# sehyun03/MulActSeg

Hardware: AMD Instinct MI355X
Metric: superpixels scored/sec (higher is better)
Workload: dtype f32; 1 GPU; acquisition-round: PixBal+ban-ignore scorer on resident logits, Cityscapes pool shape [4,20,1024,2048] per step; per rank K single-pass scans (class prior + region sums + histograms) of its shard, then exchange 1 (all-gather class sums) + device class weights (k_class_weight) + weighted finalize + ban + exchange 2 (all-gather scores) + replicated K4 (keys, radix sort, fair-counting budget walk) ov; nseg=2048, id_dtype=int64, regions_scored=679936, budget_clicks=11159, regions_selected=6688

## Files before the change

mulactseg_amd/csrc/single_pass.hip:

```cpp
#include <cstdlib>
#include "common.h"

namespace {

constexpr int kThreads = 256;
constexpr int kTileW = 256;
constexpr int kTileH = 16;
constexpr int kLogSlots = 7;
constexpr int kSlots = 1 << kLogSlots;

__device__ __forceinline__ int table_slot(int* keys, int id) {
    unsigned h = ((unsigned)id * 2654435769u) >> (32 - kLogSlots);
    for (int probe = 0; probe < kSlots; ++probe) {
        int k = __hip_atomic_load(&keys[h], __ATOMIC_RELAXED, __HIP_MEMORY_SCOPE_WORKGROUP);
        if (k == id) return (int)h;
        if (k == -1) {
            int old = atomicCAS(&keys[h], -1, id);
            if (old == -1 || old == id) return (int)h;
        }
        h = (h + 1) & (kSlots - 1);
    }
    return -1;
}

struct LowSrc { int h, w; float sh, sw; };
constexpr int kLowRows = 7, kLowCols = 68;

__device__ __forceinline__ void low_tap(float scale, int o, int& i0, float& l0, float& l1) {
    float s = scale * ((float)o + 0.5f) - 0.5f;
    s = s < 0.0f ? 0.0f : s;
    i0 = (int)s;
    l1 = s - (float)i0;
    l0 = 1.0f - l1;
}

template <int CT, bool EXACT, typename IdT, bool VEC, bool LOWRES = false, bool X4 = false>
__global__ __launch_bounds__(kThreads) void k_single_pass(const float* __restrict__ z, const IdT* __restrict__ spx, int C, int H,
                                                           int W, int S, float invT, int tiles_x, int tiles_y,
                                                           mas_u64* __restrict__ prob_sum, mas_u64* __restrict__ class_sum,
                                                           unsigned* __restrict__ hist, const LowSrc lr = LowSrc{0, 0, 0.f, 0.f}) {
    extern __shared__ __attribute__((aligned(16))) unsigned char smem[];
    mas_u64* t_sum = reinterpret_cast<mas_u64*>(smem);
    mas_u64* s_part = reinterpret_cast<mas_u64*>(smem + sizeof(mas_u64) * kSlots * C);
    unsigned* t_hist = reinterpret_cast<unsigned*>(smem + sizeof(mas_u64) * (kSlots * C + 4 * CT));
    int* t_keys = reinterpret_cast<int*>(smem + sizeof(mas_u64) * (kSlots * C + 4 * CT) + sizeof(unsigned) * kSlots * C);
    float* s_low = reinterpret_cast<float*>(t_keys + kSlots);

    for (int i = threadIdx.x; i < kSlots; i += kThreads) t_keys[i] = -1;
    for (int i = threadIdx.x; i < kSlots * C; i += kThreads) { t_sum[i] = 0; t_hist[i] = 0; }

    int bid = blockIdx.x;
    const int tx = bid % tiles_x; bid /= tiles_x;
    const int ty = bid % tiles_y;
    const int b = bid / tiles_y;
    const int HW = H * W;
    const float* zb = z + (size_t)b * C * (LOWRES ? lr.h * lr.w : HW);
    int low_r0 = 0, low_c0 = 0;
    if (LOWRES) {
        float u0, u1;
        low_tap(lr.sh, ty * kTileH, low_r0, u0, u1);
        low_tap(lr.sw, tx * kTileW, low_c0, u0, u1);
        const int lane_ = threadIdx.x & (MAS_WAVE - 1), wave_ = threadIdx.x / MAS_WAVE;
        for (int cr = wave_; cr < C * kLowRows; cr += kThreads / MAS_WAVE) {
            const int c = cr / kLowRows, r = cr - c * kLowRows;
            const int gy = min(low_r0 + r, lr.h - 1);
            const float* src = zb + ((size_t)c * lr.h + gy) * lr.w;
            for (int x = lane_; x < kLowCols; x += MAS_WAVE) s_low[cr * kLowCols + x] = src[min(low_c0 + x, lr.w - 1)];
        }
    }
    __syncthreads();
    const IdT* sb = spx + (size_t)b * HW;
    mas_u64* gsum = class_sum + (size_t)b * S * C;
    unsigned* ghist = hist + (size_t)b * S * C;
    const int lane = threadIdx.x & (MAS_WAVE - 1);
    const int wave = threadIdx.x / MAS_WAVE;

    unsigned acc[CT];
#pragma unroll
    for (int c = 0; c < CT; ++c) acc[c] = 0;
    unsigned n_quanta = 0;
    int lx[4];
    mas_v2f l0xa = mas_splat(0.f), l1xa = mas_splat(0.f), l0xb = mas_splat(0.f), l1xb = mas_splat(0.f);
    if (LOWRES) {
        float a0[4], a1[4];
#pragma unroll
        for (int k = 0; k < 4; ++k) {
            const int xk = tx * kTileW + (VEC ? (lane * 4 + k) : (k * MAS_WAVE + lane));
            int i0;
            low_tap(lr.sw, xk < W ? xk : W - 1, i0, a0[k], a1[k]);
            lx[k] = i0 - low_c0;
        }
        l0xa = (mas_v2f){a0[0], a0[1]}; l1xa = (mas_v2f){a1[0], a1[1]};
        l0xb = (mas_v2f){a0[2], a0[3]}; l1xb = (mas_v2f){a1[2], a1[3]};
    }

    for (int it = 0; it < kTileH / 4; ++it) {
        const int y = ty * kTileH + it * 4 + wave;
        if (y >= H) break;
        const size_t row = (size_t)y * W;
        int xs[4];
        bool ok[4];
#pragma unroll
        for (int k = 0; k < 4; ++k) {
            xs[k] = tx * kTileW + (VEC ? (lane * 4 + k) : (k * MAS_WAVE + lane));
            ok[k] = xs[k] < W;
        }
        int id[4];
#pragma unroll
        for (int k = 0; k < 4; ++k) {
            id[k] = ok[k] ? mas_load_id(sb, row + xs[k]) : -1;
            if (id[k] >= S) id[k] = -1;
        }
        mas_v2f v[2][CT];
        float b1[4], b2[4];
        int a1[4];
#pragma unroll
        for (int k = 0; k < 4; ++k) { b1[k] = -__builtin_inff(); b2[k] = -__builtin_inff(); a1[k] = 0; }
        int ly = 0;
        mas_v2f l0y = mas_splat(0.f), l1y = mas_splat(0.f);
        if (LOWRES) {
            float u0, u1;
            low_tap(lr.sh, y, ly, u0, u1);
            ly -= low_r0;
            l0y = mas_splat(u0);
            l1y = mas_splat(u1);
        }
        if (LOWRES) {
            if constexpr (X4) {
                mas_v2f raw[2][4];
                auto fetch4 = [&](int c, mas_v2f (&d)[4]) {
                    const float* r0 = s_low + (c * kLowRows + ly) * kLowCols;
                    const float* r1 = r0 + kLowCols;
                    d[0] = (mas_v2f){r0[lx[0]], r0[lx[0] + 1]}; d[1] = (mas_v2f){r1[lx[0]], r1[lx[0] + 1]};
                    d[2] = (mas_v2f){r0[lx[2]], r0[lx[2] + 1]}; d[3] = (mas_v2f){r1[lx[2]], r1[lx[2] + 1]};
                };
                const mas_v2f ly01 = {l0y.x, l1y.x};
                fetch4(0, raw[0]);
#pragma unroll
                for (int c = 0; c < CT; ++c) {
                    if (EXACT || c < C) {
                        if (c + 1 < CT && (EXACT || c + 1 < C)) fetch4(c + 1, raw[(c + 1) & 1]);
                        const mas_v2f (&d)[4] = raw[c & 1];
                        v[0][c] = mas_pk_mul_lo(ly01, mas_pk_mul_lo(d[0], l0xa) + mas_pk_mul_hi(d[0], l1xa))
                                + mas_pk_mul_hi(ly01, mas_pk_mul_lo(d[1], l0xa) + mas_pk_mul_hi(d[1], l1xa));
                        v[1][c] = mas_pk_mul_lo(ly01, mas_pk_mul_lo(d[2], l0xb) + mas_pk_mul_hi(d[2], l1xb))
                                + mas_pk_mul_hi(ly01, mas_pk_mul_lo(d[3], l0xb) + mas_pk_mul_hi(d[3], l1xb));
                    }
                }
            } else {
                float raw[2][16];
                auto fetch16 = [&](int c, float (&d)[16]) {
                    const float* r0 = s_low + (c * kLowRows + ly) * kLowCols;
                    const float* r1 = r0 + kLowCols;
#pragma unroll
                    for (int k = 0; k < 4; ++k) {
                        d[4 * k] = r0[lx[k]]; d[4 * k + 1] = r0[lx[k] + 1]; d[4 * k + 2] = r1[lx[k]]; d[4 * k + 3] = r1[lx[k] + 1];
                    }
                };
                fetch16(0, raw[0]);
#pragma unroll
                for (int c = 0; c < CT; ++c) {
                    if (EXACT || c < C) {
                        if (c + 1 < CT && (EXACT || c + 1 < C)) fetch16(c + 1, raw[(c + 1) & 1]);
                        const float (&d)[16] = raw[c & 1];
                        const mas_v2f v00a = {d[0], d[4]}, v01a = {d[1], d[5]}, v10a = {d[2], d[6]}, v11a = {d[3], d[7]};
                        const mas_v2f v00b = {d[8], d[12]}, v01b = {d[9], d[13]}, v10b = {d[10], d[14]}, v11b = {d[11], d[15]};
                        v[0][c] = l0y * (l0xa * v00a + l1xa * v01a) + l1y * (l0xa * v10a + l1xa * v11a);
                        v[1][c] = l0y * (l0xb * v00b + l1xb * v01b) + l1y * (l0xb * v10b + l1xb * v11b);
                    }
                }
            }
        }
#pragma unroll
        for (int c = 0; c < CT; ++c) {
            if (EXACT || c < C) {
                float4 t = make_float4(0.f, 0.f, 0.f, 0.f);
                const float* zc = zb + (size_t)c * HW;
                if (LOWRES) {
                    t = make_float4(v[0][c].x, v[0][c].y, v[1][c].x, v[1][c].y);
                } else if (VEC) {
                    if (ok[0]) t = mas_load_stream4(zc + (unsigned)(row + xs[0]));
                } else {
                    if (ok[0]) t.x = zc[row + xs[0]];
                    if (ok[1]) t.y = zc[row + xs[1]];
                    if (ok[2]) t.z = zc[row + xs[2]];
                    if (ok[3]) t.w = zc[row + xs[3]];
                }
                v[0][c] = (mas_v2f){t.x, t.y};
                v[1][c] = (mas_v2f){t.z, t.w};
                const float q[4] = {t.x, t.y, t.z, t.w};
#pragma unroll
                for (int k = 0; k < 4; ++k) {
                    const bool g1 = q[k] > b1[k];
                    b2[k] = __builtin_amdgcn_fmed3f(b1[k], b2[k], q[k]);
                    a1[k] = g1 ? c : a1[k];
                    b1[k] = __builtin_amdgcn_fmed3f(b1[k], q[k], 3.402823466e+38f);
                }
            } else {
                v[0][c] = mas_splat(0.f);
                v[1][c] = mas_splat(0.f);
            }
        }
        __builtin_amdgcn_sched_barrier(0);
        {
            mas_v2f Ra, Rb;
            mas_softmax_quad<CT, EXACT, true>(v[0], v[1], C, invT, Ra, Rb, (mas_v2f){b1[0], b1[1]}, (mas_v2f){b1[2], b1[3]});
            Ra = Ra * mas_splat(8388608.0f);
            Rb = Rb * mas_splat(8388608.0f);
            Ra = (mas_v2f){ok[0] ? Ra.x : 0.0f, ok[1] ? Ra.y : 0.0f};
            Rb = (mas_v2f){ok[2] ? Rb.x : 0.0f, ok[3] ? Rb.y : 0.0f};
#pragma unroll
            for (int c = 0; c < CT; ++c) {
                if (EXACT || c < C) {
                    const mas_v2f ta = mas_pk_fma(v[0][c], Ra, mas_splat(8388608.0f));
                    const mas_v2f tb = mas_pk_fma(v[1][c], Rb, mas_splat(8388608.0f));
                    acc[c] += (mas_f2u(ta.x) + mas_f2u(ta.y)) + (mas_f2u(tb.x) + mas_f2u(tb.y));
                }
            }
        }
        __builtin_amdgcn_sched_barrier(0);
        n_quanta += 4;
        mas_u64 q[4];
        int key[4];
        float margin[4];
        mas_bvsb_quad(b1, b2, invT, margin);
#pragma unroll
        for (int k = 0; k < 4; ++k) {
            q[k] = mas_fix_unit(margin[k]);
            key[k] = id[k] < 0 ? -1 : id[k] * MAS_MAX_CLASSES + a1[k];
        }
        const bool same = (key[0] == key[1]) && (key[1] == key[2]) && (key[2] == key[3]);
        if (same) {
            if (key[0] >= 0) {
                const int s = table_slot(t_keys, id[0]);
                const mas_u64 qs = (q[0] + q[1]) + (q[2] + q[3]);
                if (s >= 0) {
                    lds_add(&t_sum[s * C + a1[0]], qs);
                    lds_add(&t_hist[s * C + a1[0]], 4u);
                } else {
                    atomicAdd(&gsum[(size_t)id[0] * C + a1[0]], qs);
                    atomicAdd(&ghist[(size_t)id[0] * C + a1[0]], 4u);
                }
            }
        } else {
#pragma unroll
            for (int k = 0; k < 4; ++k) {
                if (key[k] < 0) continue;
                const int s = table_slot(t_keys, id[k]);
                if (s >= 0) {
                    lds_add(&t_sum[s * C + a1[k]], q[k]);
                    lds_add(&t_hist[s * C + a1[k]], 1u);
                } else {
                    atomicAdd(&gsum[(size_t)id[k] * C + a1[k]], q[k]);
                    atomicAdd(&ghist[(size_t)id[k] * C + a1[k]], 1u);
                }
            }
        }
    }

#pragma unroll
    for (int c = 0; c < CT; ++c) {
        mas_u64 a = acc[c] - n_quanta * MAS_PROBQ_BIAS;
#pragma unroll
        for (int off = MAS_WAVE / 2; off > 0; off >>= 1) a += __shfl_down(a, off, MAS_WAVE);
        if (lane == 0) s_part[wave * CT + c] = a;
    }
    __syncthreads();
    if (threadIdx.x < CT && (EXACT || (int)threadIdx.x < C)) {
        mas_u64 a = 0;
#pragma unroll
        for (int w = 0; w < kThreads / MAS_WAVE; ++w) a += s_part[w * CT + threadIdx.x];
        if (a) atomicAdd(&prob_sum[(size_t)b * C + threadIdx.x], a);
    }
    for (int i = threadIdx.x; i < kSlots * C; i += kThreads) {
        const unsigned n = t_hist[i];
        if (n) {
            const int s = i / C;
            const size_t g = (size_t)t_keys[s] * C + (i - s * C);
            atomicAdd(&ghist[g], n);
            atomicAdd(&gsum[g], t_sum[i]);
        }
    }
}

constexpr int kRingTileH = 64;
constexpr int kRingRows = kRingTileH / 4;

template <typename IdT> struct IdQuad;
template <> struct IdQuad<long long> {
    int4 a, b;
    __device__ __forceinline__ void load(const long long* p) {
        a = *reinterpret_cast<const int4*>(p);
        b = *reinterpret_cast<const int4*>(p + 2);
    }
    __device__ __forceinline__ void get(int (&id)[4]) const {
        id[0] = a.y == 0 ? a.x : -1;
        id[1] = a.w == 0 ? a.z : -1;
        id[2] = b.y == 0 ? b.x : -1;
        id[3] = b.w == 0 ? b.z : -1;
    }
};
template <> struct IdQuad<int> {
    int4 a;
    __device__ __forceinline__ void load(const int* p) { a = *reinterpret_cast<const int4*>(p); }
    __device__ __forceinline__ void get(int (&id)[4]) const { id[0] = a.x; id[1] = a.y; id[2] = a.z; id[3] = a.w; }
};
template <> struct IdQuad<unsigned short> {
    uint2 a;
    __device__ __forceinline__ void load(const unsigned short* p) { a = *reinterpret_cast<const uint2*>(p); }
    __device__ __forceinline__ void get(int (&id)[4]) const {
        id[0] = (int)(a.x & 0xffffu); id[1] = (int)(a.x >> 16); id[2] = (int)(a.y & 0xffffu); id[3] = (int)(a.y >> 16);
    }
};

template <int CT, typename IdT>
struct RowRegs {
    float4 t[CT];
    IdQuad<IdT> ids;
};

template <int CT, bool EXACT, typename IdT>
__device__ __forceinline__ void ring_issue(RowRegs<CT, IdT>& r, const float* __restrict__ zb, const IdT* __restrict__ sb, int C,
                                           int HW, unsigned off) {
    r.ids.load(sb + off);
#pragma unroll
    for (int c = 0; c < CT; ++c) {
        if (EXACT || c < C) r.t[c] = mas_load_stream4(zb + (size_t)c * HW + off);
        else r.t[c] = make_float4(0.f, 0.f, 0.f, 0.f);
    }
}

template <int CT, bool EXACT, typename IdT>
__device__ __forceinline__ void ring_consume(RowRegs<CT, IdT>& r, bool ok, int C, int S, float invT, unsigned* s_acc, int* t_keys,
                                             mas_u64* t_sum, unsigned* t_hist, mas_u64* __restrict__ gsum,
                                             unsigned* __restrict__ ghist, int& last_id, int& last_slot) {
    mas_v2f v[2][CT];
    float b1[4], b2[4];
    int a1[4];
#pragma unroll
    for (int k = 0; k < 4; ++k) { b1[k] = -__builtin_inff(); b2[k] = -__builtin_inff(); a1[k] = 0; }
#pragma unroll
    for (int c = 0; c < CT; ++c) {
        if (EXACT || c < C) {
            const float4 t = r.t[c];
            v[0][c] = (mas_v2f){t.x, t.y};
            v[1][c] = (mas_v2f){t.z, t.w};
            const float q[4] = {t.x, t.y, t.z, t.w};
#pragma unroll
            for (int k = 0; k < 4; ++k) {
                const bool g1 = q[k] > b1[k];
                b2[k] = __builtin_amdgcn_fmed3f(b1[k], b2[k], q[k]);
                a1[k] = g1 ? c : a1[k];
                b1[k] = __builtin_amdgcn_fmed3f(b1[k], q[k], 3.402823466e+38f);
            }
        } else {
            v[0][c] = mas_splat(0.f);
            v[1][c] = mas_splat(0.f);
        }
    }
    __builtin_amdgcn_sched_barrier(0);
    {
        mas_v2f Ra, Rb;
        mas_softmax_quad<CT, EXACT, true>(v[0], v[1], C, invT, Ra, Rb, (mas_v2f){b1[0], b1[1]}, (mas_v2f){b1[2], b1[3]});
        Ra = Ra * mas_splat(8388608.0f);
        Rb = Rb * mas_splat(8388608.0f);
        Ra = ok ? Ra : mas_splat(0.0f);
        Rb = ok ? Rb : mas_splat(0.0f);
#pragma unroll
        for (int c = 0; c < CT; ++c) {
            if (EXACT || c < C) {
                const mas_v2f ta = mas_pk_fma(v[0][c], Ra, mas_splat(8388608.0f));
                const mas_v2f tb = mas_pk_fma(v[1][c], Rb, mas_splat(8388608.0f));
                lds_add(&s_acc[c * kThreads + threadIdx.x], (mas_f2u(ta.x) + mas_f2u(ta.y)) + (mas_f2u(tb.x) + mas_f2u(tb.y)));
            }
        }
    }
    __builtin_amdgcn_sched_barrier(0);
    mas_u64 q[4];
    int key[4], id[4];
    float margin[4];
    r.ids.get(id);
    mas_bvsb_quad(b1, b2, invT, margin);
#pragma unroll
    for (int k = 0; k < 4; ++k) {
        id[k] = (ok && id[k] >= 0 && id[k] < S) ? id[k] : -1;
        q[k] = mas_fix_unit(margin[k]);
        key[k] = id[k] < 0 ? -1 : id[k] * MAS_MAX_CLASSES + a1[k];
    }
    const bool same = (key[0] == key[1]) && (key[1] == key[2]) && (key[2] == key[3]);
    if (same) {
        if (key[0] >= 0) {
            if (id[0] != last_id) {
                last_slot = table_slot(t_keys, id[0]);
                last_id = id[0];
            }
            const int s = last_slot;
            const mas_u64 qs = (q[0] + q[1]) + (q[2] + q[3]);
            if (s >= 0) {
                lds_add(&t_sum[s * C + a1[0]], qs);
                lds_add(&t_hist[s * C + a1[0]], 4u);
            } else {
                atomicAdd(&gsum[(size_t)id[0] * C + a1[0]], qs);
                atomicAdd(&ghist[(size_t)id[0] * C + a1[0]], 4u);
            }
        }
    } else {
#pragma unroll
        for (int k = 0; k < 4; ++k) {
            if (key[k] < 0) continue;
            const int s = table_slot(t_keys, id[k]);
            if (s >= 0) {
                lds_add(&t_sum[s * C + a1[k]], q[k]);
                lds_add(&t_hist[s * C + a1[k]], 1u);
            } else {
                atomicAdd(&gsum[(size_t)id[k] * C + a1[k]], q[k]);
                atomicAdd(&ghist[(size_t)id[k] * C + a1[k]], 1u);
            }
        }
    }
}

template <int CT, bool EXACT, typename IdT>
__global__ __launch_bounds__(kThreads, 2) void k_single_pass_ring(const float* __restrict__ z, const IdT* __restrict__ spx, int C,
                                                                   int H, int W, int S, float invT, int tiles_x, int tiles_y,
                                                                   mas_u64* __restrict__ prob_sum,
                                                                   mas_u64* __restrict__ class_sum, unsigned* __restrict__ hist) {
    extern __shared__ __attribute__((aligned(16))) unsigned char smem[];
    mas_u64* t_sum = reinterpret_cast<mas_u64*>(smem);
    mas_u64* s_part = reinterpret_cast<mas_u64*>(smem + sizeof(mas_u64) * kSlots * C);
    unsigned* t_hist = reinterpret_cast<unsigned*>(smem + sizeof(mas_u64) * (kSlots * C + 4 * CT));
    int* t_keys = reinterpret_cast<int*>(smem + sizeof(mas_u64) * (kSlots * C + 4 * CT) + sizeof(unsigned) * kSlots * C);
    unsigned* s_acc = reinterpret_cast<unsigned*>(t_keys + kSlots);

    for (int i = threadIdx.x; i < kSlots; i += kThreads) t_keys[i] = -1;
    for (int i = threadIdx.x; i < kSlots * C; i += kThreads) { t_sum[i] = 0; t_hist[i] = 0; }
#pragma unroll
    for (int c = 0; c < CT; ++c) s_acc[c * kThreads + threadIdx.x] = 0;
    __syncthreads();

    int bid = blockIdx.x;
    const int tx = bid % tiles_x; bid /= tiles_x;
    const int ty = bid % tiles_y;
    const int b = bid / tiles_y;
    const int HW = H * W;
    const float* zb = z + (size_t)b * C * HW;
    const IdT* sb = spx + (size_t)b * HW;
    mas_u64* gsum = class_sum + (size_t)b * S * C;
    unsigned* ghist = hist + (size_t)b * S * C;
    const int lane = threadIdx.x & (MAS_WAVE - 1);
    const int wave = threadIdx.x / MAS_WAVE;

    const int x0 = tx * kTileW + lane * 4;
    const bool okx = x0 < W;
    const unsigned xc = okx ? (unsigned)x0 : 0u;
    const int ybase = ty * kRingTileH + wave;
    auto off_of = [&](int it) -> unsigned {
        int y = ybase + it * 4;
        y = y < H ? y : H - 1;
        return (unsigned)y * (unsigned)W + xc;
    };
    auto ok_of = [&](int it) -> bool { return okx && (ybase + it * 4 < H); };

    RowRegs<CT, IdT> A, B;
    int last_id = -2, last_slot = -1;
    ring_issue<CT, EXACT, IdT>(A, zb, sb, C, HW, off_of(0));
#pragma unroll 1
    for (int it = 0; it < kRingRows; it += 2) {
        ring_issue<CT, EXACT, IdT>(B, zb, sb, C, HW, off_of(it + 1));
        __builtin_amdgcn_sched_barrier(0);
        ring_consume<CT, EXACT, IdT>(A, ok_of(it), C, S, invT, s_acc, t_keys, t_sum, t_hist, gsum, ghist, last_id, last_slot);
        __builtin_amdgcn_sched_barrier(0);
        ring_issue<CT, EXACT, IdT>(A, zb, sb, C, HW, off_of(it + 2 < kRingRows ? it + 2 : kRingRows - 1));
        __builtin_amdgcn_sched_barrier(0);
        ring_consume<CT, EXACT, IdT>(B, ok_of(it + 1), C, S, invT, s_acc, t_keys, t_sum, t_hist, gsum, ghist, last_id, last_slot);
        __builtin_amdgcn_sched_barrier(0);
    }

    __syncthreads();
#pragma unroll
    for (int c = 0; c < CT; ++c) {
        mas_u64 a = s_acc[c * kThreads + threadIdx.x] - (unsigned)(kRingRows * 4) * MAS_PROBQ_BIAS;
#pragma unroll
        for (int off = MAS_WAVE / 2; off > 0; off >>= 1) a += __shfl_down(a, off, MAS_WAVE);
        if (lane == 0) s_part[wave * CT + c] = a;
    }
    __syncthreads();
    if (threadIdx.x < CT && (EXACT || (int)threadIdx.x < C)) {
        mas_u64 a = 0;
#pragma unroll
        for (int w = 0; w < kThreads / MAS_WAVE; ++w) a += s_part[w * CT + threadIdx.x];
        if (a) atomicAdd(&prob_sum[(size_t)b * C + threadIdx.x], a);
    }
    for (int i = threadIdx.x; i < kSlots * C; i += kThreads) {
        const unsigned n = t_hist[i];
        if (n) {
            const int s = i / C;
            const size_t g = (size_t)t_keys[s] * C + (i - s * C);
            atomicAdd(&ghist[g], n);
            atomicAdd(&gsum[g], t_sum[i]);
        }
    }
}

__global__ __launch_bounds__(kThreads) void k_region_finalize_weighted(const mas_u64* __restrict__ class_sum,
                                                                        const unsigned* __restrict__ hist, long long n_regions,
                                                                        int C, const unsigned* __restrict__ w31, int ban_class,
                                                                        float* __restrict__ score, int* __restrict__ dominant,
                                                                        unsigned* __restrict__ count,
                                                                        long long* __restrict__ hist_i64) {
    extern __shared__ __attribute__((aligned(16))) unsigned char smem[];
    const int CP = C | 1;
    mas_u64* s_sum = reinterpret_cast<mas_u64*>(smem);
    unsigned* s_hist = reinterpret_cast<unsigned*>(s_sum + (size_t)kThreads * CP);
    const long long r0 = (long long)blockIdx.x * kThreads;
    const long long rows = (n_regions - r0) < kThreads ? (n_regions - r0) : kThreads;
    const long long words = rows * C;
    for (long long i = threadIdx.x; i < words; i += kThreads) {
        const int row = (int)(i / C), col = (int)(i - (long long)row * C);
        const unsigned hv = hist[r0 * C + i];
        s_sum[row * CP + col] = class_sum[r0 * C + i];
        s_hist[row * CP + col] = hv;
        if (hist_i64) hist_i64[r0 * C + i] = (long long)hv;
    }
    __syncthreads();
    if ((long long)threadIdx.x >= rows) return;
    const long long r = r0 + threadIdx.x;
    const unsigned* h = s_hist + threadIdx.x * CP;
    const mas_u64* cs = s_sum + threadIdx.x * CP;
    unsigned long long n = 0;
    unsigned best = 0;
    int arg = 0;
    uint64_t hi = 0, lo = 0;
    for (int c = 0; c < C; ++c) {
        const unsigned v = h[c];
        n += v;
        if (v > best) { best = v; arg = c; }
        if (v) mas_mac_u64_u32((uint64_t)cs[c], w31[c], &hi, &lo);
    }
    float sc = 0.0f;
    if (n) sc = mas_fixed_mean(mas_shr31_u128(hi, lo), n, MAS_SCORE_FRAC);
    if (ban_class >= 0 && arg == ban_class) sc = 0.0f;
    score[r] = sc;
    if (dominant) dominant[r] = arg;
    if (count) count[r] = (unsigned)n;
}

inline bool mas_ring_enabled() {
    static const bool on = [] { const char* e = getenv("MAS_SINGLE_PASS_RING"); return !(e && e[0] == '0'); }();
    return on;
}

inline size_t smem_bytes(int C, int CT) {
    return sizeof(mas_u64) * ((size_t)kSlots * C + 4 * CT) + sizeof(unsigned) * (size_t)kSlots * C + sizeof(int) * kSlots;
}

template <int CT, bool EXACT, typename IdT>
int launch(const float* z, const void* spx, int B, int C, int H, int W, int S, float invT, mas_u64* prob_sum, mas_u64* class_sum,
           unsigned* hist, hipStream_t st) {
    const int tiles_x = (W + kTileW - 1) / kTileW;
    const int tiles_y = (H + kTileH - 1) / kTileH;
    const long long nblk = (long long)B * tiles_x * tiles_y;
    if (nblk <= 0 || nblk > 0x7fffffffLL) return MAS_ERR_SHAPE;
    const bool vec = (W % 4 == 0) && (((uintptr_t)z & 15) == 0);
    const size_t smem = smem_bytes(C, CT);
    const IdT* ids = static_cast<const IdT*>(spx);
    if constexpr (EXACT) if (vec && H >= kRingTileH && (((uintptr_t)spx & 15) == 0) && mas_ring_enabled()) {
        const int rtiles_y = (H + kRingTileH - 1) / kRingTileH;
        const long long rblk = (long long)B * tiles_x * rtiles_y;
        hipLaunchKernelGGL((k_single_pass_ring<CT, EXACT, IdT>), dim3((unsigned)rblk), dim3(kThreads),
                           smem + sizeof(unsigned) * CT * kThreads, st, z, ids, C, H, W, S, invT, tiles_x, rtiles_y, prob_sum,
                           class_sum, hist);
        return mas_launch_status();
    }
    if (vec)
        hipLaunchKernelGGL((k_single_pass<CT, EXACT, IdT, true>), dim3((unsigned)nblk), dim3(kThreads), smem, st, z, ids, C, H, W, S,
                           invT, tiles_x, tiles_y, prob_sum, class_sum, hist);
    else
        hipLaunchKernelGGL((k_single_pass<CT, EXACT, IdT, false>), dim3((unsigned)nblk), dim3(kThreads), smem, st, z, ids, C, H, W, S,
                           invT, tiles_x, tiles_y, prob_sum, class_sum, hist);
    return mas_launch_status();
}

template <int CT, bool EXACT, typename IdT>
int launch_low(const float* zq, int h, int w, const void* spx, int B, int C, int H, int W, int S, float invT, mas_u64* prob_sum,
               mas_u64* class_sum, unsigned* hist, unsigned flags, hipStream_t st) {
    const int tiles_x = (W + kTileW - 1) / kTileW;
    const int tiles_y = (H + kTileH - 1) / kTileH;
    const long long nblk = (long long)B * tiles_x * tiles_y;
    if (nblk <= 0 || nblk > 0x7fffffffLL) return MAS_ERR_SHAPE;
    const LowSrc lr{h, w, (float)h / (float)H, (float)w / (float)W};
    if ((double)kTileH * h / H + 2.0 > kLowRows || (double)kTileW * w / W + 2.0 > kLowCols) return MAS_ERR_RANGE;
    const size_t smem = smem_bytes(C, CT) + sizeof(float) * (size_t)C * kLowRows * kLowCols;
    const bool vec = (W % 4 == 0);
    const IdT* ids = static_cast<const IdT*>(spx);
    static bool attr_vec[64] = {}, attr_scalar[64] = {}, attr_x4[64] = {};
    int dev = 0;
    if (hipError_t e = hipGetDevice(&dev); e != hipSuccess) return (int)e;
    const bool cached = dev >= 0 && dev < 64;
    if (vec && W == 4 * w && !(flags & MAS_LOWRES_GENERIC)) {
        if (!cached || !attr_x4[dev]) {
            const hipError_t e = hipFuncSetAttribute(reinterpret_cast<const void*>(&k_single_pass<CT, EXACT, IdT, true, true, true>),
                                                     hipFuncAttributeMaxDynamicSharedMemorySize, 128 * 1024);
            if (e != hipSuccess) return (int)e;
            if (cached) attr_x4[dev] = true;
        }
        hipLaunchKernelGGL((k_single_pass<CT, EXACT, IdT, true, true, true>), dim3((unsigned)nblk), dim3(kThreads), smem, st, zq, ids, C, H, W,
                           S, invT, tiles_x, tiles_y, prob_sum, class_sum, hist, lr);
    } else if (vec) {
        if (!cached || !attr_vec[dev]) {
            const hipError_t e = hipFuncSetAttribute(reinterpret_cast<const void*>(&k_single_pass<CT, EXACT, IdT, true, true>),
                                                     hipFuncAttributeMaxDynamicSharedMemorySize, 128 * 1024);
            if (e != hipSuccess) return (int)e;
            if (cached) attr_vec[dev] = true;
        }
        hipLaunchKernelGGL((k_single_pass<CT, EXACT, IdT, true, true>), dim3((unsigned)nblk), dim3(kThreads), smem, st, zq, ids, C, H, W, S,
                           invT, tiles_x, tiles_y, prob_sum, class_sum, hist, lr);
    } else {
        if (!cached || !attr_scalar[dev]) {
            const hipError_t e = hipFuncSetAttribute(reinterpret_cast<const void*>(&k_single_pass<CT, EXACT, IdT, false, true>),
                                                     hipFuncAttributeMaxDynamicSharedMemorySize, 128 * 1024);
            if (e != hipSuccess) return (int)e;
            if (cached) attr_scalar[dev] = true;
        }
        hipLaunchKernelGGL((k_single_pass<CT, EXACT, IdT, false, true>), dim3((unsigned)nblk), dim3(kThreads), smem, st, zq, ids, C, H, W, S,
                           invT, tiles_x, tiles_y, prob_sum, class_sum, hist, lr);
    }
    return mas_launch_status();
}

template <int CT, bool EXACT>
int dispatch_low_ids(const float* zq, int h, int w, const void* spx, int spx_dtype, int B, int C, int H, int W, int S, float invT,
                     mas_u64* prob_sum, mas_u64* class_sum, unsigned* hist, unsigned flags, hipStream_t st) {
    switch (spx_dtype) {
        case MAS_ID_I64: return launch_low<CT, EXACT, long long>(zq, h, w, spx, B, C, H, W, S, invT, prob_sum, class_sum, hist, flags, st);
        case MAS_ID_I32: return launch_low<CT, EXACT, int>(zq, h, w, spx, B, C, H, W, S, invT, prob_sum, class_sum, hist, flags, st);
        case MAS_ID_U16: return launch_low<CT, EXACT, unsigned short>(zq, h, w, spx, B, C, H, W, S, invT, prob_sum, class_sum, hist, flags, st);
        default: return MAS_ERR_DTYPE;
    }
}

template <int CT, bool EXACT>
int dispatch_ids(const float* z, const void* spx, int spx_dtype, int B, int C, int H, int W, int S, float invT, mas_u64* prob_sum,
                 mas_u64* class_sum, unsigned* hist, hipStream_t st) {
    switch (spx_dtype) {
        case MAS_ID_I64: return launch<CT, EXACT, long long>(z, spx, B, C, H, W, S, invT, prob_sum, class_sum, hist, st);
        case MAS_ID_I32: return launch<CT, EXACT, int>(z, spx, B, C, H, W, S, invT, prob_sum, class_sum, hist, st);
        case MAS_ID_U16: return launch<CT, EXACT, unsigned short>(z, spx, B, C, H, W, S, invT, prob_sum, class_sum, hist, st);
        default: return MAS_ERR_DTYPE;
    }
}

}

extern "C" int mas_single_pass_accum(const float* z, const void* spx, int spx_dtype, int B, int C, int H, int W, int S, float invT,
                                     uint64_t* prob_sum, uint64_t* class_sum, uint32_t* hist, void* stream) {
    if (!z || !spx || !prob_sum || !class_sum || !hist) return MAS_ERR_NULL;
    if (B <= 0 || H <= 0 || W <= 0 || S <= 0 || (long long)H * W > (1LL << 23)) return MAS_ERR_SHAPE;
    if (C < 2 || C > MAS_MAX_CLASSES) return MAS_ERR_CLASSES;
    hipStream_t st = static_cast<hipStream_t>(stream);
    mas_u64* ps = reinterpret_cast<mas_u64*>(prob_sum);
    mas_u64* cs = reinterpret_cast<mas_u64*>(class_sum);
    switch (C) {
        case 19: return dispatch_ids<19, true>(z, spx, spx_dtype, B, C, H, W, S, invT, ps, cs, hist, st);
        case 20: return dispatch_ids<20, true>(z, spx, spx_dtype, B, C, H, W, S, invT, ps, cs, hist, st);
        case 21: return dispatch_ids<21, true>(z, spx, spx_dtype, B, C, H, W, S, invT, ps, cs, hist, st);
        default: return dispatch_ids<MAS_MAX_CLASSES, false>(z, spx, spx_dtype, B, C, H, W, S, invT, ps, cs, hist, st);
    }
}

extern "C" int mas_single_pass_accum_lowres_opt(const float* zq, int h, int w, const void* spx, int spx_dtype, int B, int C, int H, int W, int S,
                                                float invT, uint64_t* prob_sum, uint64_t* class_sum, uint32_t* hist, unsigned flags, void* stream) {
    if (!zq || !spx || !prob_sum || !class_sum || !hist) return MAS_ERR_NULL;
    if (B <= 0 || H <= 0 || W <= 0 || S <= 0 || h <= 0 || w <= 0 || h > H || w > W || (long long)H * W > (1LL << 23)) return MAS_ERR_SHAPE;
    if (flags & ~MAS_LOWRES_GENERIC) return MAS_ERR_RANGE;
    hipStream_t st = static_cast<hipStream_t>(stream);
    mas_u64* ps = reinterpret_cast<mas_u64*>(prob_sum);
    mas_u64* cs = reinterpret_cast<mas_u64*>(class_sum);
    switch (C) {
        case 19: return dispatch_low_ids<19, true>(zq, h, w, spx, spx_dtype, B, C, H, W, S, invT, ps, cs, hist, flags, st);
        case 20: return dispatch_low_ids<20, true>(zq, h, w, spx, spx_dtype, B, C, H, W, S, invT, ps, cs, hist, flags, st);
        case 21: return dispatch_low_ids<21, true>(zq, h, w, spx, spx_dtype, B, C, H, W, S, invT, ps, cs, hist, flags, st);
        default: return MAS_ERR_CLASSES;
    }
}

extern "C" int mas_single_pass_accum_lowres(const float* zq, int h, int w, const void* spx, int spx_dtype, int B, int C, int H, int W, int S,
                                            float invT, uint64_t* prob_sum, uint64_t* class_sum, uint32_t* hist, void* stream) {
    return mas_single_pass_accum_lowres_opt(zq, h, w, spx, spx_dtype, B, C, H, W, S, invT, prob_sum, class_sum, hist, 0u, stream);
}

extern "C" int mas_region_finalize_weighted(const uint64_t* class_sum, const uint32_t* hist, int64_t n_regions, int C,
                                            const uint32_t* w31, int ban_class, float* score, int32_t* dominant, uint32_t* count,
                                            int64_t* hist_i64, void* stream) {
    if (!class_sum || !hist || !w31 || !score) return MAS_ERR_NULL;
    if (n_regions <= 0) return MAS_ERR_SHAPE;
    if (C < 1 || C > MAS_MAX_CLASSES) return MAS_ERR_CLASSES;
    const long long nblk = (n_regions + kThreads - 1) / kThreads;
    if (nblk > 0x7fffffffLL) return MAS_ERR_SHAPE;
    const size_t smem = (sizeof(mas_u64) + sizeof(unsigned)) * (size_t)kThreads * (C | 1);
    hipLaunchKernelGGL(k_region_finalize_weighted, dim3((unsigned)nblk), dim3(kThreads), smem, static_cast<hipStream_t>(stream),
                       reinterpret_cast<const mas_u64*>(class_sum), hist, (long long)n_regions, C, w31, ban_class, score, dominant,
                       count, reinterpret_cast<long long*>(hist_i64));
    return mas_launch_status();
}
```

Baseline: 55.06 million superpixels/s.

## Refill ring registers inside consume to overlap loads with softmax accumulation

The ring pipeline now issues both row buffers up front and refills each buffer channel-by-channel inside the consume step, right after that channel's value has been accumulated. The last pair of rows is peeled off without a refill. This keeps more loads in flight during compute and removes the separate issue phase and its redundant clamped reload at the tail. Smaller changes hoist id extraction ahead of the math, use byte-offset addressing for the loads, and put block indices into scalar registers via readfirstlane. The extra sched_barriers and the longer live ranges could raise register pressure or constrain the compiler's scheduling.

```diff
diff --git a/mulactseg_amd/csrc/single_pass.hip b/mulactseg_amd/csrc/single_pass.hip
--- a/mulactseg_amd/csrc/single_pass.hip
+++ b/mulactseg_amd/csrc/single_pass.hip
@@ -285,13 +285,15 @@
 
 constexpr int kRingTileH = 64;
 constexpr int kRingRows = kRingTileH / 4;
+static_assert(kRingRows >= 4 && kRingRows % 2 == 0, "the ring loop takes rows in pairs and peels the last pair");
 
 template <typename IdT> struct IdQuad;
 template <> struct IdQuad<long long> {
     int4 a, b;
-    __device__ __forceinline__ void load(const long long* p) {
+    __device__ __forceinline__ void load(const long long* base, unsigned off) {
+        const char* p = reinterpret_cast<const char*>(base) + off * 8u;
         a = *reinterpret_cast<const int4*>(p);
-        b = *reinterpret_cast<const int4*>(p + 2);
+        b = *reinterpret_cast<const int4*>(p + 16);
     }
     __device__ __forceinline__ void get(int (&id)[4]) const {
         id[0] = a.y == 0 ? a.x : -1;
@@ -302,16 +304,24 @@
 };
 template <> struct IdQuad<int> {
     int4 a;
-    __device__ __forceinline__ void load(const int* p) { a = *reinterpret_cast<const int4*>(p); }
+    __device__ __forceinline__ void load(const int* base, unsigned off) {
+        a = *reinterpret_cast<const int4*>(reinterpret_cast<const char*>(base) + off * 4u);
+    }
     __device__ __forceinline__ void get(int (&id)[4]) const { id[0] = a.x; id[1] = a.y; id[2] = a.z; id[3] = a.w; }
 };
 template <> struct IdQuad<unsigned short> {
     uint2 a;
-    __device__ __forceinline__ void load(const unsigned short* p) { a = *reinterpret_cast<const uint2*>(p); }
+    __device__ __forceinline__ void load(const unsigned short* base, unsigned off) {
+        a = *reinterpret_cast<const uint2*>(reinterpret_cast<const char*>(base) + off * 2u);
+    }
     __device__ __forceinline__ void get(int (&id)[4]) const {
         id[0] = (int)(a.x & 0xffffu); id[1] = (int)(a.x >> 16); id[2] = (int)(a.y & 0xffffu); id[3] = (int)(a.y >> 16);
     }
 };
+
+__device__ __forceinline__ float4 ring_load4(const float* plane, unsigned off) {
+    return mas_load_stream4(reinterpret_cast<const float*>(reinterpret_cast<const char*>(plane) + off * 4u));
+}
 
 template <int CT, typename IdT>
 struct RowRegs {
@@ -322,21 +332,29 @@
 template <int CT, bool EXACT, typename IdT>
 __device__ __forceinline__ void ring_issue(RowRegs<CT, IdT>& r, const float* __restrict__ zb, const IdT* __restrict__ sb, int C,
                                            int HW, unsigned off) {
-    r.ids.load(sb + off);
+    r.ids.load(sb, off);
 #pragma unroll
     for (int c = 0; c < CT; ++c) {
-        if (EXACT || c < C) r.t[c] = mas_load_stream4(zb + (size_t)c * HW + off);
+        if (EXACT || c < C) r.t[c] = ring_load4(zb + (size_t)c * HW, off);
         else r.t[c] = make_float4(0.f, 0.f, 0.f, 0.f);
     }
 }
 
-template <int CT, bool EXACT, typename IdT>
+template <int CT, bool EXACT, typename IdT, bool REFILL>
 __device__ __forceinline__ void ring_consume(RowRegs<CT, IdT>& r, bool ok, int C, int S, float invT, unsigned* s_acc, int* t_keys,
                                              mas_u64* t_sum, unsigned* t_hist, mas_u64* __restrict__ gsum,
-                                             unsigned* __restrict__ ghist, int& last_id, int& last_slot) {
+                                             unsigned* __restrict__ ghist, int& last_id, int& last_slot,
+                                             const float* __restrict__ zb, const IdT* __restrict__ sb, int HW, unsigned noff) {
     mas_v2f v[2][CT];
     float b1[4], b2[4];
-    int a1[4];
+    int a1[4], id[4];
+    r.ids.get(id);
+#pragma unroll
+    for (int k = 0; k < 4; ++k) {
+        id[k] = (ok && id[k] >= 0 && id[k] < S) ? id[k] : -1;
+        asm volatile("" : "+v"(id[k]));
+    }
+    __builtin_amdgcn_sched_barrier(0);
 #pragma unroll
     for (int k = 0; k < 4; ++k) { b1[k] = -__builtin_inff(); b2[k] = -__builtin_inff(); a1[k] = 0; }
 #pragma unroll
@@ -372,18 +390,21 @@
                 const mas_v2f ta = mas_pk_fma(v[0][c], Ra, mas_splat(8388608.0f));
                 const mas_v2f tb = mas_pk_fma(v[1][c], Rb, mas_splat(8388608.0f));
                 lds_add(&s_acc[c * kThreads + threadIdx.x], (mas_f2u(ta.x) + mas_f2u(ta.y)) + (mas_f2u(tb.x) + mas_f2u(tb.y)));
+                if constexpr (REFILL) {
+                    if (c == 0) r.ids.load(sb, noff);
+                    r.t[c] = ring_load4(zb + (size_t)c * HW, noff);
+                    __builtin_amdgcn_sched_barrier(0);
+                }
             }
         }
     }
     __builtin_amdgcn_sched_barrier(0);
     mas_u64 q[4];
-    int key[4], id[4];
+    int key[4];
     float margin[4];
-    r.ids.get(id);
     mas_bvsb_quad(b1, b2, invT, margin);
 #pragma unroll
     for (int k = 0; k < 4; ++k) {
-        id[k] = (ok && id[k] >= 0 && id[k] < S) ? id[k] : -1;
         q[k] = mas_fix_unit(margin[k]);
         key[k] = id[k] < 0 ? -1 : id[k] * MAS_MAX_CLASSES + a1[k];
     }
@@ -439,9 +460,9 @@
     __syncthreads();
 
     int bid = blockIdx.x;
-    const int tx = bid % tiles_x; bid /= tiles_x;
-    const int ty = bid % tiles_y;
-    const int b = bid / tiles_y;
+    const int tx = __builtin_amdgcn_readfirstlane(bid % tiles_x); bid /= tiles_x;
+    const int ty = __builtin_amdgcn_readfirstlane(bid % tiles_y);
+    const int b = __builtin_amdgcn_readfirstlane(bid / tiles_y);
     const int HW = H * W;
     const float* zb = z + (size_t)b * C * HW;
     const IdT* sb = spx + (size_t)b * HW;
@@ -464,17 +485,22 @@
     RowRegs<CT, IdT> A, B;
     int last_id = -2, last_slot = -1;
     ring_issue<CT, EXACT, IdT>(A, zb, sb, C, HW, off_of(0));
+    ring_issue<CT, EXACT, IdT>(B, zb, sb, C, HW, off_of(1));
+    __builtin_amdgcn_sched_barrier(0);
 #pragma unroll 1
-    for (int it = 0; it < kRingRows; it += 2) {
-        ring_issue<CT, EXACT, IdT>(B, zb, sb, C, HW, off_of(it + 1));
+    for (int it = 0; it <= kRingRows - 4; it += 2) {
+        ring_consume<CT, EXACT, IdT, true>(A, ok_of(it), C, S, invT, s_acc, t_keys, t_sum, t_hist, gsum, ghist, last_id, last_slot, zb, sb,
+                                           HW, off_of(it + 2));
         __builtin_amdgcn_sched_barrier(0);
-        ring_consume<CT, EXACT, IdT>(A, ok_of(it), C, S, invT, s_acc, t_keys, t_sum, t_hist, gsum, ghist, last_id, last_slot);
+        ring_consume<CT, EXACT, IdT, true>(B, ok_of(it + 1), C, S, invT, s_acc, t_keys, t_sum, t_hist, gsum, ghist, last_id, last_slot, zb,
+                                           sb, HW, off_of(it + 3));
         __builtin_amdgcn_sched_barrier(0);
-        ring_issue<CT, EXACT, IdT>(A, zb, sb, C, HW, off_of(it + 2 < kRingRows ? it + 2 : kRingRows - 1));
-        __builtin_amdgcn_sched_barrier(0);
-        ring_consume<CT, EXACT, IdT>(B, ok_of(it + 1), C, S, invT, s_acc, t_keys, t_sum, t_hist, gsum, ghist, last_id, last_slot);
-        __builtin_amdgcn_sched_barrier(0);
-    }
+    }
+    ring_consume<CT, EXACT, IdT, false>(A, ok_of(kRingRows - 2), C, S, invT, s_acc, t_keys, t_sum, t_hist, gsum, ghist, last_id, last_slot,
+                                        zb, sb, HW, 0u);
+    __builtin_amdgcn_sched_barrier(0);
+    ring_consume<CT, EXACT, IdT, false>(B, ok_of(kRingRows - 1), C, S, invT, s_acc, t_keys, t_sum, t_hist, gsum, ghist, last_id, last_slot,
+                                        zb, sb, HW, 0u);
 
     __syncthreads();
 #pragma unroll
```

Measured after the change: 55.85 million superpixels/s, median of 3. Within noise of the previous version (+1.4%).

## Rewrite region finalize as row-cooperative DPP reductions; simplify ring epilogue

Applied to the files above, without the earlier changes.

The weighted finalize kernel no longer stages 256 rows through LDS with one thread per region. It now assigns a 16-lane row group to each region, with each lane owning two classes loaded as coalesced pairs, and reduces the 128-bit weighted sum (split into 27-bit limbs), count, max and argmax using DPP row shuffles. This is meant to remove the LDS staging, the divides in the copy loop and the serial per-class loop, at the cost of many DPP ops and limb arithmetic. The single-pass ring epilogue also swaps the per-wave shuffle reduction for lane-wise partial sums plus LDS atomics, and the dead final prefetch now points at a fixed address.

```diff
diff --git a/mulactseg_amd/csrc/single_pass.hip b/mulactseg_amd/csrc/single_pass.hip
--- a/mulactseg_amd/csrc/single_pass.hip
+++ b/mulactseg_amd/csrc/single_pass.hip
@@ -427,13 +427,14 @@
                                                                    mas_u64* __restrict__ class_sum, unsigned* __restrict__ hist) {
     extern __shared__ __attribute__((aligned(16))) unsigned char smem[];
     mas_u64* t_sum = reinterpret_cast<mas_u64*>(smem);
-    mas_u64* s_part = reinterpret_cast<mas_u64*>(smem + sizeof(mas_u64) * kSlots * C);
+    mas_u64* s_tot = reinterpret_cast<mas_u64*>(smem + sizeof(mas_u64) * kSlots * C);
     unsigned* t_hist = reinterpret_cast<unsigned*>(smem + sizeof(mas_u64) * (kSlots * C + 4 * CT));
     int* t_keys = reinterpret_cast<int*>(smem + sizeof(mas_u64) * (kSlots * C + 4 * CT) + sizeof(unsigned) * kSlots * C);
     unsigned* s_acc = reinterpret_cast<unsigned*>(t_keys + kSlots);
 
     for (int i = threadIdx.x; i < kSlots; i += kThreads) t_keys[i] = -1;
     for (int i = threadIdx.x; i < kSlots * C; i += kThreads) { t_sum[i] = 0; t_hist[i] = 0; }
+    if (threadIdx.x < CT) s_tot[threadIdx.x] = 0;
 #pragma unroll
     for (int c = 0; c < CT; ++c) s_acc[c * kThreads + threadIdx.x] = 0;
     __syncthreads();
@@ -460,6 +461,8 @@
         return (unsigned)y * (unsigned)W + xc;
     };
     auto ok_of = [&](int it) -> bool { return okx && (ybase + it * 4 < H); };
+    const int ylast = ybase + (kRingRows - 1) * 4;
+    const unsigned off_dead = (unsigned)(ylast < H ? ylast : H - 1) * (unsigned)W + (unsigned)(tx * kTileW);
 
     RowRegs<CT, IdT> A, B;
     int last_id = -2, last_slot = -1;
@@ -470,25 +473,31 @@
         __builtin_amdgcn_sched_barrier(0);
         ring_consume<CT, EXACT, IdT>(A, ok_of(it), C, S, invT, s_acc, t_keys, t_sum, t_hist, gsum, ghist, last_id, last_slot);
         __builtin_amdgcn_sched_barrier(0);
-        ring_issue<CT, EXACT, IdT>(A, zb, sb, C, HW, off_of(it + 2 < kRingRows ? it + 2 : kRingRows - 1));
+        ring_issue<CT, EXACT, IdT>(A, zb, sb, C, HW, it + 2 < kRingRows ? off_of(it + 2) : off_dead);
         __builtin_amdgcn_sched_barrier(0);
         ring_consume<CT, EXACT, IdT>(B, ok_of(it + 1), C, S, invT, s_acc, t_keys, t_sum, t_hist, gsum, ghist, last_id, last_slot);
         __builtin_amdgcn_sched_barrier(0);
     }
 
     __syncthreads();
-#pragma unroll
-    for (int c = 0; c < CT; ++c) {
-        mas_u64 a = s_acc[c * kThreads + threadIdx.x] - (unsigned)(kRingRows * 4) * MAS_PROBQ_BIAS;
-#pragma unroll
-        for (int off = MAS_WAVE / 2; off > 0; off >>= 1) a += __shfl_down(a, off, MAS_WAVE);
-        if (lane == 0) s_part[wave * CT + c] = a;
+    constexpr int kWaves = kThreads / MAS_WAVE;
+    unsigned w4[(CT + kWaves - 1) / kWaves][4];
+#pragma unroll
+    for (int i = 0; i < (CT + kWaves - 1) / kWaves; ++i) {
+        const int c = min(wave + i * kWaves, CT - 1);
+#pragma unroll
+        for (int k = 0; k < 4; ++k) w4[i][k] = s_acc[c * kThreads + k * MAS_WAVE + lane];
+    }
+#pragma unroll
+    for (int i = 0; i < (CT + kWaves - 1) / kWaves; ++i) {
+        const int c = wave + i * kWaves;
+        const unsigned bias = (unsigned)(kRingRows * 4) * MAS_PROBQ_BIAS;
+        const mas_u64 a = ((mas_u64)(w4[i][0] - bias) + (mas_u64)(w4[i][1] - bias)) + ((mas_u64)(w4[i][2] - bias) + (mas_u64)(w4[i][3] - bias));
+        if (c < CT) lds_add(&s_tot[c], a);
     }
     __syncthreads();
     if (threadIdx.x < CT && (EXACT || (int)threadIdx.x < C)) {
-        mas_u64 a = 0;
-#pragma unroll
-        for (int w = 0; w < kThreads / MAS_WAVE; ++w) a += s_part[w * CT + threadIdx.x];
+        const mas_u64 a = s_tot[threadIdx.x];
         if (a) atomicAdd(&prob_sum[(size_t)b * C + threadIdx.x], a);
     }
     for (int i = threadIdx.x; i < kSlots * C; i += kThreads) {
@@ -502,46 +511,109 @@
     }
 }
 
-__global__ __launch_bounds__(kThreads) void k_region_finalize_weighted(const mas_u64* __restrict__ class_sum,
+template <int CTRL>
+__device__ __forceinline__ unsigned row_peer(unsigned v) { return (unsigned)__builtin_amdgcn_update_dpp(0, (int)v, CTRL, 0xf, 0xf, false); }
+__device__ __forceinline__ void row_sum(unsigned& v) {
+    v += row_peer<0xB1>(v); v += row_peer<0x4E>(v); v += row_peer<0x141>(v); v += row_peer<0x128>(v);
+}
+__device__ __forceinline__ unsigned row_max(unsigned v) {
+    v = max(v, row_peer<0xB1>(v)); v = max(v, row_peer<0x4E>(v)); v = max(v, row_peer<0x141>(v)); return max(v, row_peer<0x128>(v));
+}
+__device__ __forceinline__ unsigned row_min(unsigned v) {
+    v = min(v, row_peer<0xB1>(v)); v = min(v, row_peer<0x4E>(v)); v = min(v, row_peer<0x141>(v)); return min(v, row_peer<0x128>(v));
+}
+
+template <bool PAIRS>
+__global__ __launch_bounds__(kThreads, PAIRS ? 4 : 3) void k_region_finalize_weighted(const mas_u64* __restrict__ class_sum,
                                                                         const unsigned* __restrict__ hist, long long n_regions,
                                                                         int C, const unsigned* __restrict__ w31, int ban_class,
                                                                         float* __restrict__ score, int* __restrict__ dominant,
                                                                         unsigned* __restrict__ count,
                                                                         long long* __restrict__ hist_i64) {
-    extern __shared__ __attribute__((aligned(16))) unsigned char smem[];
-    const int CP = C | 1;
-    mas_u64* s_sum = reinterpret_cast<mas_u64*>(smem);
-    unsigned* s_hist = reinterpret_cast<unsigned*>(s_sum + (size_t)kThreads * CP);
-    const long long r0 = (long long)blockIdx.x * kThreads;
-    const long long rows = (n_regions - r0) < kThreads ? (n_regions - r0) : kThreads;
-    const long long words = rows * C;
-    for (long long i = threadIdx.x; i < words; i += kThreads) {
-        const int row = (int)(i / C), col = (int)(i - (long long)row * C);
-        const unsigned hv = hist[r0 * C + i];
-        s_sum[row * CP + col] = class_sum[r0 * C + i];
-        s_hist[row * CP + col] = hv;
-        if (hist_i64) hist_i64[r0 * C + i] = (long long)hv;
-    }
-    __syncthreads();
-    if ((long long)threadIdx.x >= rows) return;
-    const long long r = r0 + threadIdx.x;
-    const unsigned* h = s_hist + threadIdx.x * CP;
-    const mas_u64* cs = s_sum + threadIdx.x * CP;
-    unsigned long long n = 0;
-    unsigned best = 0;
-    int arg = 0;
-    uint64_t hi = 0, lo = 0;
-    for (int c = 0; c < C; ++c) {
-        const unsigned v = h[c];
-        n += v;
-        if (v > best) { best = v; arg = c; }
-        if (v) mas_mac_u64_u32((uint64_t)cs[c], w31[c], &hi, &lo);
-    }
+    const int lane = threadIdx.x & (MAS_WAVE - 1);
+    const int j = lane & 15;
+    const long long r0 = (long long)blockIdx.x * kThreads + __builtin_amdgcn_readfirstlane((int)(threadIdx.x & ~(MAS_WAVE - 1)));
+    if (r0 >= n_regions) return;
+    const int rows = (int)((n_regions - r0) < MAS_WAVE ? (n_regions - r0) : MAS_WAVE);
+    const mas_u64* cs = class_sum + r0 * C;
+    const unsigned* hs = hist + r0 * C;
+    long long* ho = hist_i64 ? hist_i64 + r0 * C : nullptr;
+    const int c0 = 2 * j;
+    const bool in0 = c0 < C, in1 = c0 + 1 < C;
+    const unsigned wa = in0 ? w31[c0] : 0u, wb = in1 ? w31[c0 + 1] : 0u;
+
+    constexpr int kTrips = MAS_WAVE / 8;
+    unsigned n_lo = 0, n_hi = 0, arg = 0, l0 = 0, l1 = 0, l2 = 0, l3 = 0;
+#pragma unroll 1
+    for (int t0 = 0; t0 < 2 * kTrips; t0 += kTrips) {
+        uint2 hv[kTrips];
+        mas_u64 sa[kTrips], sb[kTrips];
+#pragma unroll
+        for (int t = 0; t < kTrips; ++t) {
+            const int row = (lane & 48) + t0 + t;
+            const bool live0 = in0 && row < rows, live1 = in1 && row < rows;
+            const unsigned o = (unsigned)(row * C + c0);
+            if (PAIRS) {
+                hv[t] = *reinterpret_cast<const uint2*>(hs + (live0 ? o : 0u));
+                const ulonglong2 q = *reinterpret_cast<const ulonglong2*>(cs + (live0 ? o : 0u));
+                sa[t] = q.x; sb[t] = q.y;
+            } else {
+                hv[t] = make_uint2(hs[live0 ? o : 0u], hs[live1 ? o + 1u : 0u]);
+                sa[t] = cs[live0 ? o : 0u];
+                sb[t] = cs[live1 ? o + 1u : 0u];
+            }
+            hv[t].x = live0 ? hv[t].x : 0u;
+            hv[t].y = live1 ? hv[t].y : 0u;
+        }
+
+#pragma unroll
+        for (int t = 0; t < kTrips; ++t) {
+            const int row = (lane & 48) + t0 + t;
+            const unsigned o = (unsigned)(row * C + c0);
+            const unsigned va = hv[t].x, vb = hv[t].y;
+            if (ho && row < rows) {
+                if (PAIRS) {
+                    if (in0) *reinterpret_cast<longlong2*>(ho + o) = make_longlong2((long long)va, (long long)vb);
+                } else {
+                    if (in0) ho[o] = (long long)va;
+                    if (in1) ho[o + 1u] = (long long)vb;
+                }
+            }
+            uint64_t hi = 0, lo = 0;
+            mas_mac_u64_u32(va ? (uint64_t)sa[t] : 0u, wa, &hi, &lo);
+            mas_mac_u64_u32(vb ? (uint64_t)sb[t] : 0u, wb, &hi, &lo);
+            const unsigned m27 = (1u << 27) - 1u;
+            unsigned q0 = (unsigned)lo & m27;
+            unsigned q1 = (unsigned)(lo >> 27) & m27;
+            unsigned q2 = (unsigned)((lo >> 54) | (hi << 10)) & m27;
+            unsigned q3 = (unsigned)(hi >> 17);
+            const mas_u64 nn = (mas_u64)va + vb;
+            unsigned p0 = (unsigned)nn & 0xffffffu, p1 = (unsigned)(nn >> 24);
+            unsigned best = va > vb ? va : vb;
+            row_sum(q0); row_sum(q1); row_sum(q2); row_sum(q3); row_sum(p0); row_sum(p1);
+            best = row_max(best);
+            unsigned a = va == best ? (unsigned)c0 : (vb == best ? (unsigned)c0 + 1u : 64u);
+            a = row_min(a);
+            const bool mine = j == t0 + t;
+            l0 = mine ? q0 : l0; l1 = mine ? q1 : l1; l2 = mine ? q2 : l2; l3 = mine ? q3 : l3;
+            n_lo = mine ? p0 : n_lo; n_hi = mine ? p1 : n_hi;
+            arg = mine ? a : arg;
+        }
+    }
+
+    if (lane >= rows) return;
+    const long long r = r0 + lane;
+    uint64_t lo = (uint64_t)l0 + ((uint64_t)l1 << 27);
+    uint64_t hi = ((uint64_t)l2 >> 10) + ((uint64_t)l3 << 17);
+    const uint64_t m = (uint64_t)l2 << 54;
+    lo += m;
+    hi += lo < m ? 1u : 0u;
+    const unsigned long long n = (unsigned long long)n_lo + ((unsigned long long)n_hi << 24);
     float sc = 0.0f;
     if (n) sc = mas_fixed_mean(mas_shr31_u128(hi, lo), n, MAS_SCORE_FRAC);
-    if (ban_class >= 0 && arg == ban_class) sc = 0.0f;
+    if (ban_class >= 0 && (int)arg == ban_class) sc = 0.0f;
     score[r] = sc;
-    if (dominant) dominant[r] = arg;
+    if (dominant) dominant[r] = (int)arg;
     if (count) count[r] = (unsigned)n;
 }
 
@@ -697,9 +769,14 @@
     if (C < 1 || C > MAS_MAX_CLASSES) return MAS_ERR_CLASSES;
     const long long nblk = (n_regions + kThreads - 1) / kThreads;
     if (nblk > 0x7fffffffLL) return MAS_ERR_SHAPE;
-    const size_t smem = (sizeof(mas_u64) + sizeof(unsigned)) * (size_t)kThreads * (C | 1);
-    hipLaunchKernelGGL(k_region_finalize_weighted, dim3((unsigned)nblk), dim3(kThreads), smem, static_cast<hipStream_t>(stream),
-                       reinterpret_cast<const mas_u64*>(class_sum), hist, (long long)n_regions, C, w31, ban_class, score, dominant,
-                       count, reinterpret_cast<long long*>(hist_i64));
+    const bool pairs = C % 2 == 0 && ((uintptr_t)class_sum & 15) == 0 && ((uintptr_t)hist & 7) == 0 && ((uintptr_t)hist_i64 & 15) == 0;
+    if (pairs)
+        hipLaunchKernelGGL(k_region_finalize_weighted<true>, dim3((unsigned)nblk), dim3(kThreads), 0, static_cast<hipStream_t>(stream),
+                           reinterpret_cast<const mas_u64*>(class_sum), hist, (long long)n_regions, C, w31, ban_class, score,
+                           dominant, count, reinterpret_cast<long long*>(hist_i64));
+    else
+        hipLaunchKernelGGL(k_region_finalize_weighted<false>, dim3((unsigned)nblk), dim3(kThreads), 0, static_cast<hipStream_t>(stream),
+                           reinterpret_cast<const mas_u64*>(class_sum), hist, (long long)n_regions, C, w31, ban_class, score,
+                           dominant, count, reinterpret_cast<long long*>(hist_i64));
     return mas_launch_status();
 }
```

New measurement: 55.14 million superpixels/s before, 57.71 million superpixels/s after (median of 6 runs). +4.7%, better.
